# zpaq/zpaq

Hardware: AMD Instinct MI355X
Metric: compress MB/s + bit-identical ratio, -m5 over 1024x1 MiB blocks (higher is better)
Workload: dtype int32

## Files before the change

### profiles/unit_isa.py

```python
#!/usr/bin/env python3
import collections, os, re, subprocess, sys, tempfile
ROOT = os.path.dirname(os.path.dirname(os.path.abspath(__file__)))
sys.path.insert(0, ROOT)


def classify(op):
    if op.startswith("s_waitcnt"): return "s_waitcnt"
    if op.startswith("s_nop"): return "s_nop"
    if op.startswith(("s_cbranch", "s_branch", "s_setpc", "s_swappc", "s_call")): return "branch"
    if op.startswith(("global_", "buffer_", "flat_", "scratch_")): return "vmem"
    if op.startswith("ds_"): return "lds"
    if op.startswith("s_load") or op.startswith("s_buffer"): return "smem"
    if op.startswith("s_"): return "salu"
    if op.startswith("v_"): return "valu"
    return "other"


def main():
    import zpaq_amd as z
    from zpaq_amd import corpus, prebuild
    method = sys.argv[1] if len(sys.argv) > 1 else "3"
    kind = sys.argv[2] if len(sys.argv) > 2 else "lcg"
    bs = int(sys.argv[3]) if len(sys.argv) > 3 else 1 << 18
    mode = int(sys.argv[4]) if len(sys.argv) > 4 else 0
# ... 4 lines not shown
    src, key = prebuild.pipe_source_and_key(header, mode)
    inc = os.path.join(ROOT, "zpaq_amd", "csrc", "device")
    with tempfile.TemporaryDirectory() as td:
        hip = os.path.join(td, "k.hip")
        open(hip, "w").write(src)
        subprocess.run([prebuild.HIPCC, "--offload-arch=gfx950", "-O3", "-std=c++17", "-Wno-unused-label", "-mllvm",
                        "-simplifycfg-sink-common=false", "-I", inc, "--genco", hip, "-o", os.path.join(td, "k.hsaco"),
                        "-save-temps"], cwd=td, check=True, stdout=subprocess.DEVNULL, stderr=subprocess.DEVNULL)
        asm = open(os.path.join(td, "k-hip-amdgcn-amd-amdhsa-gfx950.s")).read()
    names = {0: "HCOMP", 1: "ROW", 2: "light", 3: "ICM map", 4: "ISSE map", 5: "MIX"}
    lk = re.search(r"LIGHT_KIND\[\d+\] = \{([^}]*)\}", src)
    light_kinds = [int(x) for x in lk.group(1).split(",")] if lk else []
    lname = {2: "CONS", 3: "CM", 4: "MATCH", 5: "AVG", 6: "MIX2", 7: "SSE", 8: "CODER", 9: "CM bits", 10: "MIX2 bits", 11: "SSE bits"}
    print(f"chain of method {method} ({kind}, {bs} B blocks), n = {header[6]} components, shape {mode}; key {key}")
    print(f"{'unit':28s} {'loop':>6s} {'per bit':>8s}   valu  salu  vmem   lds  wait  branch  nop   (instructions of the per-byte loop nest, static, all paths)")
    for m in re.finditer(r"^(_ZN3zpq17pipe_persist_unitIN7zpq_gen6ChainPELi(\d+)ELi(\d+)EEEvRKNS_8PipeArgsEjii):[^\n]*\n(.*?)^\.Lfunc_end", asm, re.S | re.M):
        kindn, role, body = int(m.group(2)), int(m.group(3)), m.group(4)
        lines = body.split("\n")
        heads = [(i, int(re.search(r"Depth=(\d+)", l).group(1))) for i, l in enumerate(lines) if "Loop Header: Depth=" in l]
        best = None
        for hi, (i, d) in enumerate(heads):
            if d < 2:
                continue
            j = next((i2 for i2, d2 in heads[hi + 1:] if d2 <= d), len(lines))
            ops = [l.split()[0] for l in lines[i:j] if re.match(r"^\s+[a-z_0-9]+(\s|$)", l) and not l.strip().startswith((";", "."))]
            if best is None or len(ops) > len(best[0]):
                best = (ops, d)
        if best is None:
            continue
        ops = best[0]
        c = collections.Counter(classify(o) for o in ops)
        tag = names.get(kindn, "?")
        if kindn == 2 and role < len(light_kinds):
            tag = lname.get(light_kinds[role], "light")
        print(f"{tag + ' (role %d)' % role:28s} {len(ops):6d} {len(ops) / 8:8.1f}   {c['valu']:4d}  {c['salu']:4d}  {c['vmem']:4d}  {c['lds']:4d}  {c['s_waitcnt']:4d}  {c['branch']:6d}  {c['s_nop']:3d}")


if __name__ == "__main__":
    main()
```

### zpaq_amd/csrc/device/pipe_kernel.h

```cpp
#pragma once
#ifndef ZPQ_LANE_VM
#define ZPQ_LANE_VM 1
#endif
#include "spec_kernel.h"

namespace zpq {

typedef __attribute__((address_space(1))) short g_i16;
typedef __attribute__((address_space(1))) unsigned short g_u16;

#ifdef ZPQ_TRACE
struct PipeTraceScope {
  unsigned long long* rec;
  __device__ __forceinline__ PipeTraceScope(const PipeArgs& a, int kernel) : rec(nullptr) {
    if (a.trace && threadIdx.x == 0) {
      rec = a.trace + 4ull * ((unsigned long long)a.trace_base + blockIdx.x);
      unsigned hw, xcc;
      asm volatile("s_getreg_b32 %0, hwreg(HW_REG_HW_ID)" : "=s"(hw));
      asm volatile("s_getreg_b32 %0, hwreg(HW_REG_XCC_ID)" : "=s"(xcc));
      rec[0] = ((unsigned long long)(unsigned)kernel << 56) | ((unsigned long long)((unsigned)a.step & 0xFFFFFFu) << 32) |
               (unsigned long long)(blockIdx.x + a.wg0);
      rec[1] = ((unsigned long long)xcc << 32) | hw;
      rec[2] = __builtin_amdgcn_s_memrealtime();
    }
// ... 125 lines not shown
  __device__ __forceinline__ g_u128& p(int i, unsigned k) const {
    return *(g_u128*)(gb + (unsigned)Chain::PIPE_OFF_P + ((((slot * N + i) * C + k) * G + gl) << 4));
  }
  __device__ __forceinline__ g_u32& state(int w) const {
    return *(g_u32*)(gb + (unsigned)Chain::PIPE_OFF_STATE + (((unsigned)w * G + gl) << 2));
  }
  __device__ __forceinline__ unsigned off_ctx(int ci, unsigned k) const { return (unsigned)Chain::PIPE_OFF_CTX + ((((slot * Chain::PIPE_NCTX + ci) * C + k) * G + gl) << 2); }
  __device__ __forceinline__ unsigned off_bh(int ri, unsigned k) const { return (unsigned)Chain::PIPE_OFF_BH + ((((slot * Chain::PIPE_NROW + ri) * C + k) * G + gl) << 3); }
  __device__ __forceinline__ unsigned off_p(int i, unsigned k) const { return (unsigned)Chain::PIPE_OFF_P + ((((slot * N + i) * C + k) * G + gl) << 4); }
  __device__ __forceinline__ void put_ctx(int ci, unsigned k, unsigned v) const {
    if constexpr (WT) pipe_wt_store4(gb, off_ctx(ci, k), v); else ctx(ci, k) = v;
  }
  __device__ __forceinline__ void put_bh(int ri, unsigned k, const uint2& v) const {
    if constexpr (WT) pipe_wt_store8(gb, off_bh(ri, k), v); else bh(ri, k) = v;
  }
  __device__ __forceinline__ void put_bh_half(int ri, unsigned k, unsigned half, unsigned v) const {
    if constexpr (WT) pipe_wt_store4(gb, off_bh(ri, k) + 4u * half, v); else *(g_u32*)(gb + off_bh(ri, k) + 4u * half) = v;
  }
  __device__ __forceinline__ void put_p(int i, unsigned k, const uint4& v) const {
    if constexpr (WT) pipe_wt_store16(gb, off_p(i, k), v); else p(i, k) = v;
  }
  __device__ __forceinline__ void put_p64(int i, unsigned k, unsigned half, const uint2& v) const {
    if constexpr (WT) pipe_wt_store8(gb, off_p(i, k) + 8u * half, v); else *(g_u64v*)((g_u8*)&p(i, k) + 8u * half) = v;
  }
  __device__ __forceinline__ void put_p16(int i, unsigned k, unsigned B, int v) const {
    if constexpr (WT) pipe_wt_store2(gb, off_p(i, k) + 2u * B, (unsigned)v & 0xFFFFu); else *(g_i16*)((g_u8*)&p(i, k) + 2u * B) = (short)v;
  }
  __device__ __forceinline__ void put_state(int w, unsigned v) const {
    if constexpr (WT) pipe_wt_store4(gb, (unsigned)Chain::PIPE_OFF_STATE + (((unsigned)w * G + gl) << 2), v); else state(w) = v;
  }
  __device__ __forceinline__ g_u32& A32(unsigned off) const { return *(g_u32*)(arena + off); }
  __device__ __forceinline__ g_u8& A8(unsigned off) const { return *(g_u8*)(arena + off); }
  __device__ __forceinline__ g_u128& A128(unsigned off) const { return *(g_u128*)(arena + off); }
  __device__ __forceinline__ unsigned byte_at(unsigned k) const { return in[k0 + k]; }
  __device__ __forceinline__ unsigned next(unsigned k) const { return min(k + 1u, nb - 1u); }
};

__device__ __forceinline__ int pipe_p_get(const uint4& v, int B) {
  const unsigned w = B < 2 ? v.x : (B < 4 ? v.y : (B < 6 ? v.z : v.w));
  return (int)(short)(unsigned short)(w >> (16 * (B & 1)));
}
struct PipeP8 {
  unsigned w[4] = {0, 0, 0, 0};
  __device__ __forceinline__ void set(int B, int v) { w[B >> 1] |= ((unsigned)v & 0xFFFFu) << (16 * (B & 1)); }
  __device__ __forceinline__ uint4 get() const { return make_uint4(w[0], w[1], w[2], w[3]); }
};
// ... 1798 lines not shown
  __shared__ PipeSquash squash;
  const int lane = threadIdx.x & 63;
  const unsigned ngroups = (a.nblocks + Chain::PIPE_G - 1u) / Chain::PIPE_G;
  const unsigned wg = blockIdx.x + a.wg0;
  squash.load(a.tb, lane);
  __syncthreads();
  static_for<0, Chain::NMIXR>([&](auto rc) __attribute__((always_inline)) {
    constexpr int r = decltype(rc)::value;
    constexpr int I = Chain::MIX_COMP[r], QL = Chain::MIX_QL[r], first = Chain::MIX_FIRST[r];
    constexpr int PPW = 64 / QL, BPW = PPW / 8;
    static_assert(QL <= 8 && BPW >= 1 && (int)Chain::PIPE_G % BPW == 0, "MIX bit lanes: a block's 8 positions share a wavefront");
    constexpr int WPG = (int)Chain::PIPE_G / BPW;
    if (wg < (unsigned)first * ngroups || wg >= (unsigned)(first + WPG) * ngroups) return;
    const unsigned wi = wg - (unsigned)first * ngroups;
    const unsigned g = wi / (unsigned)WPG, sub = wi % (unsigned)WPG;
    const unsigned pair = (unsigned)lane / QL, q = (unsigned)lane % QL, B = pair & 7u;
    PipeLane<Chain> L;
    L.open(a, pipe_opaque(g * Chain::PIPE_G + sub * BPW + (pair >> 3)), Chain::P_LEVEL[I]);
    if (L.chunk < 0 || !pipe_any(L.nb > 0)) return;
    pipe_mix_bits_unit<Chain, r>(L, q, B, squash);
  });
}

template <class Chain, int r, int NH, class SQ>
__device__ __forceinline__ void pipe_mix_unit(PipeLane<Chain>& L, unsigned q, unsigned half, const SQ& squash) {
  constexpr int I = Chain::MIX_COMP[r], QL = Chain::MIX_QL[r];
  constexpr CompK c = Chain::comp[I];
  constexpr int m = (int)c.a3, J = (int)c.a2, ci = Chain::P_CTX[I];
  constexpr int NQ = (m + 3) / 4, TAIL = m % 4, NB = 8 / NH;
  static_assert(NQ <= QL, "MIX lane group");
  constexpr bool batch = c.a5 == 255u && c.mask0 >= 255u;
  static_assert(NH == 1 || (NH == 2 && batch), "a byte is split over lane groups only when its 8 rows are distinct");
  if (!L.nb) return;
  constexpr bool FULL = c.stride >= 4u * (unsigned)QL;
  const bool act = FULL || q < (unsigned)NQ;
  const bool tail = !FULL && TAIL != 0 && q == (unsigned)(NQ - 1);
  const unsigned qoff = 16u * (act ? q : 0u);
  bool have[4];
  int tin[4];
#pragma unroll
  for (int x = 0; x < 4; ++x) {
    const int t = (int)q * 4 + x;
    have[x] = t < m;
    tin[x] = J + (have[x] ? t : 0);
  }
  auto c8_of = [&](unsigned bytev, int b) __attribute__((always_inline)) -> unsigned {
    if constexpr (NH == 1) return pipe_c8(bytev, b);
    else return ((half ? 16u : 1u) << b) | ((half ? bytev : bytev >> 4) >> (4 - b));
  };
  auto y_of = [&](unsigned bytev, int b) __attribute__((always_inline)) -> int {
    if constexpr (NH == 1) return pipe_y(bytev, b);
    else return (int)(((half ? bytev : bytev >> 4) >> (3 - b)) & 1u);
  };
  auto row_of = [&](unsigned hh, unsigned bytev, int b) __attribute__((always_inline)) -> unsigned {
    return (unsigned)c.t0 + 4u * __umul24((hh + (c8_of(bytev, b) & c.a5)) & c.mask0, (unsigned)c.stride) + qoff;
  };
  unsigned h = L.ctx(ci, 0), byte = L.byte_at(0);
  const unsigned k1 = L.next(0);
  unsigned h1 = L.ctx(ci, k1), byte1 = L.byte_at(k1);
  auto inputs = [&](int x, unsigned kk) __attribute__((always_inline)) -> uint4 {
    const uint4 v = L.p(tin[x], kk);
    const unsigned mk = have[x] ? 0xFFFFFFFFu : 0u;
    if constexpr (NH == 1) return make_uint4(v.x & mk, v.y & mk, v.z & mk, v.w & mk);
    else return make_uint4((half ? v.z : v.x) & mk, (half ? v.w : v.y) & mk, 0u, 0u);
  };
  uint4 pv[4], pv1[4];
#pragma unroll
  for (int x = 0; x < 4; ++x) { pv[x] = inputs(x, 0); pv1[x] = inputs(x, k1); }
  uint4 w[NB];
  unsigned rowc[NB];
#pragma unroll
  for (int B = 0; B < NB; ++B) rowc[B] = row_of(h, byte, B);
  if constexpr (batch) {
#pragma unroll
    for (int B = 0; B < NB; ++B) w[B] = *(g_u128a4*)(L.arena + rowc[B]);
  }
  for (unsigned k = 0; k < L.nb; ++k) {
    const unsigned k2 = min(k + 2u, L.nb - 1u);
    const unsigned h2 = L.ctx(ci, k2), byte2 = L.byte_at(k2);
    uint4 pv2[4];
#pragma unroll
    for (int x = 0; x < 4; ++x) pv2[x] = inputs(x, k2);
    unsigned rown[NB];
#pragma unroll
    for (int B = 0; B < NB; ++B) rown[B] = row_of(h1, byte1, B);
    const bool same = h1 == h;
    const bool late = !same && (((h1 - h) & c.mask0) < 256u || ((h - h1) & c.mask0) < 256u);
    uint4 wn[NB], nw[NB];
    if constexpr (batch) {
      if (!late) {
#pragma unroll
        for (int B = 0; B < NB; ++B) wn[B] = *(g_u128a4*)(L.arena + rown[B]);
      }
    }
    PipeP8 out;
#pragma unroll
    for (int B = 0; B < NB; ++B) {
      const unsigned row = rowc[B];
      if constexpr (!batch) w[B] = *(g_u128a4*)(L.arena + row);
      const int w0 = (int)w[B].x, w1 = (int)w[B].y, w2 = (int)w[B].z, w3 = (int)w[B].w;
      const int p0 = pipe_p_get(pv[0], B), p1 = pipe_p_get(pv[1], B), p2 = pipe_p_get(pv[2], B), p3 = pipe_p_get(pv[3], B);
      const int dot = __mul24(w0 >> 8, p0) + __mul24(w1 >> 8, p1) + __mul24(w2 >> 8, p2) + __mul24(w3 >> 8, p3);
      const int pr = sp_clamp2k(pipe_group_sum<QL>(dot) >> 8);
      out.set(B, pr);
      const int err = __mul24(y_of(byte, B) * 32767 - squash(pr), (int)c.a4) >> 4;
      nw[B].x = (unsigned)sp_clamp512k(w0 + ((__mul24(err, p0) + (1 << 12)) >> 13));
      nw[B].y = (unsigned)sp_clamp512k(w1 + ((__mul24(err, p1) + (1 << 12)) >> 13));
      nw[B].z = (unsigned)sp_clamp512k(w2 + ((__mul24(err, p2) + (1 << 12)) >> 13));
      nw[B].w = (unsigned)sp_clamp512k(w3 + ((__mul24(err, p3) + (1 << 12)) >> 13));
      if constexpr (FULL) *(g_u128a4*)(L.arena + row) = nw[B];
      else if (act && !tail) *(g_u128a4*)(L.arena + row) = nw[B];
      if constexpr (TAIL != 0 && !FULL) {
        if (tail) {
          L.A32(row) = nw[B].x;
          if constexpr (TAIL >= 2) L.A32(row + 4u) = nw[B].y;
          if constexpr (TAIL >= 3) L.A32(row + 8u) = nw[B].z;
        }
      }
    }
    if (q == 0) {
      if constexpr (NH == 1) L.put_p(I, k, out.get());
      else L.put_p64(I, k, half, make_uint2(out.w[0], out.w[1]));
    }
    if constexpr (batch) {
      if constexpr (NH == 2) {
        if (pipe_any(late)) pipe_stores_done();
      }
      if (late) {
#pragma unroll
        for (int B = 0; B < NB; ++B) wn[B] = *(g_u128a4*)(L.arena + rown[B]);
      }
#pragma unroll
      for (int B = 0; B < NB; ++B) {
        const bool fw = same && rown[B] == rowc[B];
        w[B].x = fw ? nw[B].x : wn[B].x; w[B].y = fw ? nw[B].y : wn[B].y;
        w[B].z = fw ? nw[B].z : wn[B].z; w[B].w = fw ? nw[B].w : wn[B].w;
      }
    }
    h = h1; byte = byte1; h1 = h2; byte1 = byte2;
#pragma unroll
    for (int B = 0; B < NB; ++B) rowc[B] = rown[B];
#pragma unroll
    for (int x = 0; x < 4; ++x) { pv[x] = pv1[x]; pv1[x] = pv2[x]; }
  }
}

struct PipeW3 { unsigned x, y, z; };
typedef __attribute__((address_space(1))) PipeW3 g_w3;

__device__ __forceinline__ int pipe_sext24(unsigned v) { return (int)(v << 8) >> 8; }
__device__ __forceinline__ void pipe_unpack4(const PipeW3& d, int& w0, int& w1, int& w2, int& w3) {
  w0 = pipe_sext24(d.x);
  w1 = pipe_sext24((d.x >> 24) | (d.y << 8));
  w2 = pipe_sext24((d.y >> 16) | (d.z << 16));
  w3 = (int)d.z >> 8;
}
__device__ __forceinline__ PipeW3 pipe_pack4(int w0, int w1, int w2, int w3) {
  PipeW3 d;
  d.x = ((unsigned)w0 & 0xFFFFFFu) | ((unsigned)w1 << 24);
  d.y = (((unsigned)w1 >> 8) & 0xFFFFu) | ((unsigned)w2 << 16);
  d.z = (((unsigned)w2 >> 16) & 0xFFu) | ((unsigned)w3 << 8);
  return d;
}

__device__ __forceinline__ constexpr unsigned pipe_mix_pstride(unsigned m) {
  const unsigned need = 12u * ((m + 3u) / 4u);
// ... 200 lines not shown
```

### zpaq_amd/csrc/device/pipe_persist.h

```cpp
#pragma once
#include "pipe_kernel.h"

#if !defined(ZPQ_EMU)
#ifndef ZPQ_PERSIST_LDS_BYTES
#error "the generated source defines ZPQ_PERSIST_LDS_BYTES before it includes pipe_persist.h"
#endif
namespace zpq { __shared__ __attribute__((aligned(16))) unsigned char persist_lds[ZPQ_PERSIST_LDS_BYTES]; }
#endif

namespace zpq {

struct PipeRO {
  int dt[1024];
  unsigned short dt2k[256];
  PipeSquash squash;
  PipeStretch stretch;
  unsigned char ns[1024];
};

#ifdef ZPQ_EMU
#define ZPQ_PERSIST_LDS(bytes) ((unsigned char*)emu::wg_lds(bytes))
__device__ __forceinline__ unsigned pipe_prog_load(const unsigned* p) { return *(volatile const unsigned*)p; }
__device__ __forceinline__ void pipe_prog_add(unsigned* p) { *(volatile unsigned*)p = *(volatile unsigned*)p + 1u; }
__device__ __forceinline__ void pipe_flag_set(unsigned* p, unsigned v) { *(volatile unsigned*)p = v; }
// ... 104 lines not shown

template <class Chain>
__device__ __forceinline__ void pipe_publish(unsigned* prog, int unit, int lane) {
  pipe_drain_stores();
  if (lane == 0) pipe_prog_add(prog + unit);
}

template <class Chain, int kind, int role>
__device__ __attribute__((noinline)) void pipe_persist_unit(const PipeArgs& a, unsigned g, int lane, int SLOT) {
  unsigned char* const lds = ZPQ_PERSIST_LDS(Chain::PS_LDS_BYTES);
  const PipeRO& ro = *(const PipeRO*)lds;
  const int sub = Chain::PS_SUB[SLOT], unit = Chain::PS_UNIT[SLOT];
  constexpr unsigned G = Chain::PIPE_G;
  unsigned* const prog = pipe_uniform(a.prog + (unsigned long long)g * (unsigned)Chain::PS_NUNIT);
  const unsigned nchunks = a.group_chunks[g];
  unsigned char* const priv = lds + Chain::PS_LDS[SLOT];
  PipeLane<Chain> L;
  unsigned q = 0, B = 0, mix_bl = 0;
  if constexpr (kind == 0) {
    constexpr int HL = Chain::HCOMP_LANES < (int)G ? Chain::HCOMP_LANES : (int)G;
    const bool mine = lane < HL;
    L.bind(a, g, (unsigned)sub * HL + (mine ? (unsigned)lane : 0u), mine);
  } else if constexpr (kind == 5) {
    constexpr int QL = Chain::MIX_QL[role];
    if constexpr (Chain::MIX_BITS != 0) {
      constexpr int BPW = 64 / QL / 8;
      const unsigned pair = (unsigned)lane / QL;
      q = (unsigned)lane % QL; B = pair & 7u;
      L.bind(a, g, pipe_opaque((unsigned)sub * BPW + (pair >> 3)), true);
    } else {
      constexpr int NH = Chain::PS_MIX_NH;
      constexpr int BPW = 64 / (QL * NH) < (int)G ? 64 / (QL * NH) : (int)G;
      const unsigned bl = (unsigned)lane / (QL * NH);
      q = (unsigned)lane % QL; B = ((unsigned)lane / QL) % NH;
      mix_bl = bl;
      const bool okl = bl < (unsigned)BPW;
      L.bind(a, g, (unsigned)sub * BPW + (okl ? bl : 0u), okl);
    }
  } else if constexpr (kind == 2 && Chain::LIGHT_KIND[role < 0 ? 0 : role] >= PK_CM_BITS) {
    B = (unsigned)lane & 7u;
    const unsigned gl = (unsigned)sub * 8u + ((unsigned)lane >> 3);
    L.bind(a, g, gl < G ? gl : 0u, gl < G);
  } else if constexpr (kind == 1 && pipe_row_in_halves<Chain>(role < 0 ? 0 : role)) {
    L.bind(a, g, (unsigned)lane & 31u, true);
  } else {
    const bool okl = (unsigned)lane < G;
    L.bind(a, g, okl ? (unsigned)lane : 0u, okl);
  }
  if (!L.live) L.idle();
  L.gb = pipe_uniform(L.gb);
  unsigned long long t_wait = 0, t_work = 0, t_mark = a.trace ? pipe_clock() : 0ull;
  for (unsigned c = 0; c < nchunks; ++c) {
    if (!pipe_wait<Chain>(a, prog, c, lane, SLOT)) return;
// ... 17 lines not shown
        }
        if (pipe_any(L.nb > 0)) pipe_icm_unit<Chain, Chain::ICM_COMP[role], PipeStretchFull, PipeAhead<Chain>::value>(L, (unsigned*)priv, PipeStretchFull{st}, lane, c == 0, false);
      } else {
        if (pipe_any(L.nb > 0)) pipe_icm_unit<Chain, Chain::ICM_COMP[role], PipeStretch, PipeAhead<Chain>::value>(L, (unsigned*)priv, ro.stretch, lane, c == 0, false);
      }
    } else if constexpr (kind == 4) {
      if constexpr (PipeSmallChain<Chain>::value) {
        unsigned short* const sq = (unsigned short*)(priv + 512u * G * 4u);
        if (c == 0) {
          for (int i = lane; i < 4096; i += 64) sq[i] = a.tb->squash[i];
          (void)pipe_any(true);
        }
        if (pipe_any(L.nb > 0)) pipe_isse_unit<Chain, Chain::ISSE_COMP[role], PipeSquashFull, PipeAhead<Chain>::value>(L, (unsigned*)priv, PipeSquashFull{sq}, lane, c == 0, false);
      } else {
        if (pipe_any(L.nb > 0)) pipe_isse_packed_unit<Chain, Chain::ISSE_COMP[role], PipeSquash, PipeAhead<Chain>::value>(L, (unsigned*)priv, ro.squash, lane, c == 0);
      }
    } else if constexpr (kind == 5) {
      if (pipe_any(L.nb > 0)) {
        if constexpr (Chain::MIX_BITS != 0) pipe_mix_bits_unit<Chain, role>(L, q, B, ro.squash);
        else if constexpr (PipeMixPacked<Chain>::of(role)) {
          constexpr int QL = Chain::MIX_QL[role], NH = Chain::PS_MIX_NH, BPW = 64 / (QL * NH) < (int)G ? 64 / (QL * NH) : (int)G;
          pipe_mix_packed_unit<Chain, role, PipeMixLdsRows<Chain>::of(role), BPW, NH>(L, q, B, mix_bl < (unsigned)BPW ? mix_bl : 0u, (unsigned*)priv, c == 0, ro.squash);
        }
        else pipe_mix_unit<Chain, role, Chain::PS_MIX_NH>(L, q, B, ro.squash);
      }
    } else {
      constexpr int lk = Chain::LIGHT_KIND[role], I = Chain::LIGHT_COMP[role];
      if constexpr (lk == PK_CODER) {
        if constexpr (PipeCoderFast<Chain>::value) pipe_coder_fast<Chain, (PipeAhead<Chain>::value > 0 ? PipeAhead<Chain>::value : 1)>(L, a, (unsigned*)priv, lane, c == 0);
        else pipe_coder<Chain>(L, a, ro.squash);
      } else if (pipe_any(L.nb > 0)) {
        if constexpr (lk == PK_CONS) pipe_cons<Chain, I>(L);
        else if constexpr (lk == PK_CM) {
          if constexpr (pipe_light_lds_words<Chain>(lk, I) != 0u) pipe_cm_lds<Chain, I>(L, (unsigned*)priv, ro.stretch, ro.dt, lane, c == 0);
          else pipe_cm<Chain, I>(L, ro.stretch, ro.dt);
        }
        else if constexpr (lk == PK_MATCH) pipe_match_any<Chain, I>(L, ro.stretch, ro.dt2k);
        else if constexpr (lk == PK_AVG) pipe_avg<Chain, I>(L);
        else if constexpr (lk == PK_MIX2) {
          if constexpr (pipe_light_lds_words<Chain>(lk, I) != 0u) pipe_mix2_lds<Chain, I>(L, (unsigned*)priv, ro.squash, lane, c == 0);
          else pipe_mix2<Chain, I>(L, ro.squash);
        }
        else if constexpr (lk == PK_SSE) pipe_sse<Chain, I>(L, ro.stretch, ro.dt);
        else if constexpr (lk == PK_CM_BITS) pipe_cm_bits<Chain, I>(L, B, ro.stretch, ro.dt);
        else if constexpr (lk == PK_MIX2_BITS) pipe_mix2_bits<Chain, I>(L, B, ro.squash);
        else if constexpr (lk == PK_SSE_BITS) pipe_sse_bits<Chain, I>(L, B, ro.stretch, ro.dt);
      }
// ... 42 lines not shown
```

### zpaq_amd/csrc/host/codegen.cpp

```cpp
#include "codegen.hpp"

#include <cstdio>
#include <cstdlib>
#include <cstring>
#include <map>
#include <mutex>
#include <set>
#include <sstream>
#include <algorithm>

namespace zpq {

namespace {

struct Insn { int pc, len, op; };

std::string src_expr(int k, int imm) {
  switch (k) {
    case 0: return "a";
    case 1: return "b";
    case 2: return "c";
    case 3: return "d";
    case 4: return "(unsigned)M[b & MMASK]";
    case 5: return "(unsigned)M[c & MMASK]";
// ... 264 lines not shown
       "extern \"C\" __global__ __launch_bounds__(64 * zpq_gen::Chain::WAVES) void zpq_spec_decode(const zpq::BlockJob* jobs, "
       "zpq::BlockResult* res, unsigned nblocks, const zpq::DeviceTables* tb) {\n"
       "  " << body << "<zpq_gen::Chain, true>(jobs, res, nblocks, tb);\n}\n";
  source = o.str();
  return true;
}

PipeOptions pipe_options(int variant) {
  PipeOptions o;
  o.mode = variant ? 1 : 0;
  o.chunk = variant == 2 ? 2048 : 0;
  o.wide = variant == 3;
  return o;
}

static const int kPersistRoBytes = 4096 + 512 + 2688 + (2016 * 4 + 512) + 1024;
static const int kPersistLdsCap = 163840 - 512;
static uint32_t mix_pstride(uint32_t m) {
  const uint32_t need = 12u * ((m + 3u) / 4u);
  uint32_t p = 16u;
  while (p < need) p *= 2u;
  return p;
}
static void plan_persistent(const zpq_plan& plan, PipeLayout& L, int lds_rows_wish, bool halves) {
  const CompDesc* comp = plan.comps();
  const PlanHeader& ph = plan.hdr();
  const int n = L.n, G = L.G;
  enum { K_CONS = 2, K_CM, K_MATCH, K_AVG, K_MIX2, K_SSE, K_CODER, K_CM_BITS, K_MIX2_BITS, K_SSE_BITS };
  L.persist_ok = false;
  L.ps_slots.clear(); L.ps_deps.clear();
  int nunit = 1;
  std::vector<int> row_unit(n, -1), p_unit(n, -1);
  for (int i = 0; i < n; ++i) {
    if (L.row[i] >= 0) row_unit[i] = nunit++;
    p_unit[i] = nunit++;
  }
  const int coder_unit = nunit++;
  L.ps_nunit = nunit;
  std::vector<int> unit_waves(nunit, 0);
  std::vector<PipeLayout::Slot> slots;
  static const float ondie_w = [] { const char* v = getenv("ZPAQ_AMD_PACK_ONDIE_WEIGHT"); return v ? (float)atof(v) : 1.0f; }();
  static const float stream_w = [] { const char* v = getenv("ZPAQ_AMD_PACK_STREAM_WEIGHT"); return v ? (float)atof(v) : 1.0f; }();
  static const float match_lines = [] { const char* v = getenv("ZPAQ_AMD_PACK_MATCH_LINES"); return v ? (float)atof(v) : 3.0f; }();
  const float ctx_l = G * 4 / 128.f, bh_l = G * 8 / 128.f, p_l = G * 16 / 128.f;
  auto add = [&](int kind, int role, int sub, int unit, int lds, float cost, float lines = 0.f, float stream_lines = 0.f) {
    PipeLayout::Slot s; s.kind = kind; s.role = role; s.sub = sub; s.unit = unit; s.lds = (lds + 255) & ~255; s.cost = cost;
    s.lines = lines + stream_w * stream_lines;
// ... 37 lines not shown
    int code_role = (int)r;
    for (size_t r2 = 0; r2 < r; ++r2) if (L.light[r2] == L.light[r]) { code_role = (int)r2; break; }
    int lds = 0;
    if ((k == K_CM || (k == K_MIX2 && comp[i].mask0 != 0u)) && comp[i].mask0 + 1u <= 512u && comp[i].mask0 >= 3u) lds = (int)(comp[i].mask0 + 1u) * G * 4;
    float lines = 0.f;
    if (!lds) {
      const float wcm = line_weight(4ull * (comp[i].mask0 + 1ull));
      if (k == K_CM) lines = 2.f * G * wcm;
      else if (k == K_CM_BITS) lines = 2.f * 8 * wcm;
      else if (k == K_MATCH) lines = match_lines * G;
      else if (k == K_MIX2 && comp[i].mask0 != 0u) lines = 8.f * G * wcm;
      else if (k == K_MIX2_BITS) lines = 8.f * 8 * wcm;
      else if (k == K_SSE) lines = 8.f * G * wcm;
      else if (k == K_SSE_BITS) lines = 8.f * 8 * wcm;
    }
    const bool bits = k >= K_CM_BITS;
    float sl = (k == K_CODER ? p_l : p_l + ctx_l) + (k == K_MIX2 || k == K_MIX2_BITS || k == K_AVG ? 2.f * p_l : (k == K_SSE || k == K_SSE_BITS ? p_l : 0.f));
    if (bits) sl *= 8.f * 8.f / (float)(G * 8);
    if (k == K_CODER && L.ps_coder_fast) lds = 4096 * 4;
    add(2, code_role, L.light_sub[r], k == K_CODER ? coder_unit : p_unit[i], lds, lds && k != K_CODER ? 0.9f : lc[k < 12 ? k : 0], lines, sl);
  }
  for (size_t r = 0; r < L.icm.size(); ++r) add(3, (int)r, 0, p_unit[L.icm[r]], 256 * G * 4 + (small && L.ps_icm_full ? 65536 : 0), 1.1f, 0.f, bh_l + p_l);
  for (size_t r = 0; r < L.isse.size(); ++r) add(4, (int)r, 0, p_unit[L.isse[r]], small ? 512 * G * 4 + 8192 : 256 * G * 4 + 64 * G * 4, 1.5f, 0.f, bh_l + 2.f * p_l);
  L.ps_mix_nh = 1;
  if (halves && !L.mix_bits && !L.mix.empty()) {
    bool ok = true;
    for (size_t r = 0; r < L.mix.size(); ++r) {
      const CompDesc& c = comp[L.mix[r]];
      ok = ok && c.a5 == 255u && c.mask0 >= 255u && L.mix_ql[r] * 2 <= 64;
    }
    if (ok) L.ps_mix_nh = 2;
  }
  L.mix_lds_rows.assign(L.mix.size(), 0);
  for (size_t r = 0; r < L.mix.size(); ++r) {
    const int nw = L.mix_bits ? L.mix_waves_of(L.mix_ql[r]) : std::max(1, G * L.mix_ql[r] * L.ps_mix_nh / 64);
    int lds = 0;
    const CompDesc& c = comp[L.mix[r]];
    if (!L.mix_bits && L.mix_packed[r] && c.mask0 + 1u <= 256u && lds_rows_wish > 0) {
      const int rows = std::min<int>(lds_rows_wish, (int)(c.mask0 + 1u));
      const int nq = ((int)c.a3 + 3) / 4, bpw = std::max(1, std::min(G, 64 / (L.mix_ql[r] * L.ps_mix_nh)));
      L.mix_lds_rows[r] = rows;
      lds = 3 * rows * nq * bpw * 4;
    }
    const float groups_per_wave = 64.f / (float)L.mix_ql[r];
    float lines = groups_per_wave * (L.mix_bits ? 1.f : 8.f / (float)L.ps_mix_nh) * line_weight(4ull * c.stride * (c.mask0 + 1ull));
    if (L.mix_lds_rows[r]) lines *= 1.f / 8.f;
    for (int sub = 0; sub < nw; ++sub)
      add(5, (int)r, sub, p_unit[L.mix[r]], lds, L.mix_bits ? 0.55f : (L.ps_mix_nh == 2 ? 1.7f : (lds ? 1.6f : 2.6f)), lines, (float)c.a3 + ctx_l);
  }
  std::vector<std::vector<int>> producers(nunit);
  auto reads = [&](int u, int v) { if (u != v && std::find(producers[u].begin(), producers[u].end(), v) == producers[u].end()) producers[u].push_back(v); };
  for (int i = 0; i < n; ++i) {
    const CompDesc& c = comp[i];
    const int u = p_unit[i];
    if (L.row[i] >= 0) { reads(row_unit[i], 0); reads(u, row_unit[i]); }
    else if (L.ctx[i] >= 0) reads(u, 0);
    switch (c.type) {
      case C_ISSE: reads(u, p_unit[c.a2]); break;
      case C_AVG: reads(u, p_unit[c.a1]); reads(u, p_unit[c.a2]); break;
      case C_MIX2: reads(u, p_unit[c.a2]); reads(u, p_unit[c.a3]); break;
      case C_SSE: reads(u, p_unit[c.a2]); break;
      case C_MIX: for (unsigned t = 0; t < c.a3; ++t) reads(u, p_unit[c.a2 + t]); break;
      default: break;
    }
  }
  reads(coder_unit, p_unit[n - 1]);
  reads(coder_unit, 0);
  std::vector<std::vector<PipeLayout::Dep>> unit_deps(nunit);
  for (int u = 0; u < nunit; ++u)
    for (int v : producers[u]) {
      unit_deps[u].push_back({v, 0, unit_waves[v]});
// ... 235 lines not shown
  L.coder_state = L.nstate; L.nstate += 4;
  const uint64_t hbytes = 4ull * (ph.hmask + 1);
  L.hcomp_h_lds = hbytes <= 8192;
  L.hcomp_lanes = 64;
  if (L.hcomp_h_lds) while (L.hcomp_lanes > 8 && hbytes * L.hcomp_lanes > 65536) L.hcomp_lanes /= 2;
  const uint64_t C = (uint64_t)L.C, S = (uint64_t)L.S, G = (uint64_t)L.G;
  uint64_t off = 0;
  L.off_ctx = off;   off += S * (uint64_t)std::max(L.nctx, 1) * C * G * 4;
  L.off_bh = off;    off += S * (uint64_t)std::max(L.nrow, 1) * C * G * 8;
  L.off_p = off;     off += S * (uint64_t)n * C * G * 16;
  L.off_state = off; off += (uint64_t)L.nstate * G * 4;
  L.group_bytes = (off + 4095) & ~4095ull;
  if (L.group_bytes >= (1ull << 32)) { why_not = "stream buffer of a block group exceeds 4 GiB"; return false; }
  L.mix_packed.assign(L.mix.size(), 0);
  static const bool packed_off = [] { const char* v = getenv("ZPAQ_AMD_MIX_PACKED"); return !(v && v[0] == '1'); }();
  for (size_t r = 0; r < L.mix.size(); ++r) {
    const CompDesc& c = comp[L.mix[r]];
    const uint32_t ps = mix_pstride(c.a3);
    if (!packed_off && !L.mix_bits && c.a5 == 255u && c.mask0 >= 255u && c.a3 >= 3u && ps <= 4u * c.stride && (ps < 4u * c.stride || c.mask0 + 1u <= 256u))
      L.mix_packed[r] = 1;
  }
  static const int rows_forced = [] { const char* v = getenv("ZPAQ_AMD_MIX_LDS_ROWS"); return v ? atoi(v) : -1; }();
  static const bool halves_wanted = [] { const char* v = getenv("ZPAQ_AMD_MIX_HALVES"); return !(v && v[0] == '0'); }();
  plan_persistent(plan, L, 0, false);
  bool halves = false;
  if (L.persist_ok && halves_wanted) {
    PipeLayout T = L;
    plan_persistent(plan, T, 0, true);
    if (T.persist_ok && T.ps_mix_nh == 2 && T.ps_wpg <= L.ps_wpg) { L = T; halves = true; }
  }
  if (L.persist_ok) {
    const int wpg0 = L.ps_wpg;
    for (int wish : {128, 64, 32}) {
      if (rows_forced >= 0 && wish != rows_forced) continue;
      PipeLayout T = L;
      plan_persistent(plan, T, wish, halves);
      bool any = false;
      for (int v : T.mix_lds_rows) any = any || v != 0;
      if (!any) break;
      if (T.persist_ok && T.ps_wpg <= wpg0) { L = T; break; }
    }
  }
  return true;
}

bool generate_pipe_source(const zpq_plan& plan, const PipeOptions& opt, std::string& source, std::string& why_not) {
  PipeLayout L;
  if (!pipe_layout(plan, opt, L, why_not)) return false;
  const PlanHeader& ph = plan.hdr();
  const int n = L.n;
  const CompDesc* comp = plan.comps();
  std::ostringstream o;
  o << "// generated by zpaq_amd codegen v" << kCodegenVersion << " (pipelined encoder) -- do not edit\n"
       "#define ZPQ_PERSIST_LDS_BYTES " << (L.persist_ok && opt.persist && opt.chunk != 2048 ? L.ps_lds_bytes : 16) << "\n"
       "#include \"pipe_persist.h\"\n"
       "namespace zpq_gen {\n"
       "struct Chain {\n";
  int nmix = 0, nsse = 0;
  std::ostringstream comps;
// ... 63 lines not shown
         "  static constexpr bool PIPE_PERSIST = true;\n"
         "  static constexpr int PS_MIX_NH = " << L.ps_mix_nh << ";\n"
         "  static constexpr bool HCOMP_M_LDS = " << (L.hcomp_m_lds ? "true" : "false") << ";\n"
         "  static constexpr int PS_AHEAD = " << L.ps_ahead << ";\n"
         "  static constexpr bool PS_ROW_RING = " << (L.ps_row_ring ? "true" : "false") << ";\n"
         "  static constexpr bool PS_CODER_FAST = " << (L.ps_coder_fast ? "true" : "false") << ", PS_SMALL = " << (L.ps_small ? "true" : "false") << ";\n"
      << (L.ps_small && !L.ps_row_halves ? "  static constexpr bool PS_ROW_HALVES = false;\n" : "")
      << (L.ps_small && !L.ps_icm_full ? "  static constexpr bool PS_ICM_FULL = false;\n" : "")
      << "";
    o <<
         "  static constexpr int PS_WAVES = " << L.ps_waves << ", PS_WPG = " << L.ps_wpg << ", PS_NSLOT = " << L.ps_slots.size()
      << ", PS_NUNIT = " << L.ps_nunit << ", PS_LDS_BYTES = " << L.ps_lds_bytes << ";\n";
    arr("PS_KIND", kind.data(), (int)kind.size());
    arr("PS_ROLE", role.data(), (int)role.size());
    arr("PS_SUB", sub.data(), (int)sub.size());
    arr("PS_UNIT", unit.data(), (int)unit.size());
    arr("PS_LDS", ldso.data(), (int)ldso.size());
    arr("PS_DEP0", dep0.data(), (int)dep0.size());
    arr("PS_NDEP", ndep.data(), (int)ndep.size());
    arr("PS_DEP_UNIT", du.data(), (int)du.size());
    arr("PS_DEP_LAG", dl.data(), (int)dl.size());
    arr("PS_DEP_MULT", dm.data(), (int)dm.size());
    arr("MIX_LDS_ROWS", L.mix_lds_rows.data(), (int)L.mix_lds_rows.size());
    o << "};\n";
  }
  o << "}  // namespace zpq_gen\n";
  if (L.persist_ok && opt.persist && opt.chunk != 2048)
    o << "extern \"C\" __global__ __launch_bounds__(" << 64 * L.ps_waves << ") void zpq_pipe_persist(zpq::PipeArgs a) {\n"
         "  zpq::pipe_persist_body<zpq_gen::ChainP>(a);\n}\n";
  else
    o << "#ifdef ZPQ_EMU\nextern \"C\" void zpq_pipe_persist(zpq::PipeArgs) {}\n#endif\n";
  o << "extern \"C\" __global__ __launch_bounds__(256) void zpq_pipe_repack(zpq::PipeArgs a) {\n"
       "  zpq::pipe_repack_body<zpq_gen::Chain>(a);\n}\n";
  const char* names[6] = {"hcomp", "rows", "light", "icm", "isse", "mix"};
  for (int k = 0; k < 6; ++k)
    o << "extern \"C\" __global__ __launch_bounds__(64) void zpq_pipe_" << names[k] << "(zpq::PipeArgs a) {\n"
         "  ZPQ_PIPE_TRACE(a, " << k << ");\n"
         "  zpq::pipe_" << names[k] << "_body<zpq_gen::Chain>(a);\n}\n";
  source = o.str();
  return true;
}

bool generate_pcomp_source(const U8* code, size_t len, int ph, int pm, std::string& source, std::string& why_not) {
  if (len < 1 || len > 65535) { why_not = "empty or oversized PCOMP"; return false; }
  if (ph > 28 || pm > 30) { why_not = "PCOMP arrays too large"; return false; }
  std::ostringstream o;
// ... 25 lines not shown
```

### zpaq_amd/csrc/host/codegen.hpp

```cpp
#pragma once
#include <string>
#include <utility>
#include <vector>

#include "../device/plan.hpp"
#include "common.hpp"

namespace zpq {

static const int kCodegenVersion = 6;

bool generate_spec_source(const zpq_plan& plan, int waves, std::string& source, std::string& why_not, int shape = 0);
int team_threads(const zpq_plan& plan);

struct PipeOptions {
  int mode = 0;
  int chunk = 0;
  int group = 0;
  bool persist = true;
  bool wide = false;
};
static const int kPipeVariants = 4;
PipeOptions pipe_options(int variant);

// ... 25 lines not shown
    int role = 0;
    int sub = 0;
    int unit = 0;
    int lds = 0;
    int lds_off = 0;
    float cost = 0;
    float lines = 0;
  };
  struct Dep { int unit, lag, mult; };
  bool persist_ok = false;
  std::string persist_why;
  int ps_waves = 0;
  int ps_wpg = 0;
  int ps_nunit = 0;
  int ps_lds_bytes = 0;
  bool ps_coder_fast = false;
  bool ps_row_ring = false;
  int ps_ahead = 0;
  bool ps_wide = false;
  bool ps_icm_full = false;
  bool ps_row_halves = false;
  bool ps_small = false;
  int ps_mix_nh = 1;
  std::vector<Slot> ps_slots;
  std::vector<std::vector<Dep>> ps_deps;
  int light_threads() const { return 64; }
  int mix_waves_of(int ql) const { return mix_bits ? G * ql / 8 : ql; }
  int mix_waves_per_group() const { int s = 0; for (int q : mix_ql) s += mix_waves_of(q); return s; }
  int mix_threads() const { return mix_bits ? 64 : G; }
};
bool pipe_layout(const zpq_plan& plan, const PipeOptions& opt, PipeLayout& out, std::string& why_not);
bool generate_pipe_source(const zpq_plan& plan, const PipeOptions& opt, std::string& source, std::string& why_not);

bool generate_pcomp_source(const U8* code, size_t len, int ph, int pm, std::string& source, std::string& why_not);

std::string spec_cache_key(const std::string& source);

}
```

Before: 386.9.

## Split MIX bytes over four lane groups and allow five weights per lane

The persistent pipeline's MIX unit can now split each byte's 8 bit-rows across four lane groups instead of two. It can also give each lane five weights instead of four when that halves the lane group and the padded row stride allows it. The planner tries NH=4 first, then NH=2, and emits per-role lane-group sizes and words-per-lane tables. This aims to shorten each lane's serial bit chain and cut the lanes spent per mixer. The cost is extra 32-bit partial stores of predictions and more units to schedule. The unit_isa profiling script is also changed to find loop extents more precisely and skip spin-wait loops.

```diff
diff --git a/profiles/unit_isa.py b/profiles/unit_isa.py
--- a/profiles/unit_isa.py
+++ b/profiles/unit_isa.py
@@ -50,8 +50,14 @@
         for hi, (i, d) in enumerate(heads):
             if d < 2:
                 continue
-            j = next((i2 for i2, d2 in heads[hi + 1:] if d2 <= d), len(lines))
+            name = next((re.match(r"^\.L(BB\d+_\d+):", lines[k]).group(1) for k in range(i, max(i - 4, -1), -1) if re.match(r"^\.LBB\d+_\d+:", lines[k])), None)
+            if name is None:
+                continue
+            last = max((k for k, l in enumerate(lines) if re.search(r"(Header=|Parent Loop )%s\b" % name, l)), default=i)
+            j = next((k for k in range(last + 1, len(lines)) if re.match(r"^(\.LBB\d+_\d+:|; %bb\.\d+:)", lines[k])), len(lines))
             ops = [l.split()[0] for l in lines[i:j] if re.match(r"^\s+[a-z_0-9]+(\s|$)", l) and not l.strip().startswith((";", "."))]
+            if "s_sleep" in ops:
+                continue
             if best is None or len(ops) > len(best[0]):
                 best = (ops, d)
         if best is None:
diff --git a/zpaq_amd/csrc/device/pipe_kernel.h b/zpaq_amd/csrc/device/pipe_kernel.h
--- a/zpaq_amd/csrc/device/pipe_kernel.h
+++ b/zpaq_amd/csrc/device/pipe_kernel.h
@@ -171,6 +171,9 @@
   }
   __device__ __forceinline__ void put_p64(int i, unsigned k, unsigned half, const uint2& v) const {
     if constexpr (WT) pipe_wt_store8(gb, off_p(i, k) + 8u * half, v); else *(g_u64v*)((g_u8*)&p(i, k) + 8u * half) = v;
+  }
+  __device__ __forceinline__ void put_p32(int i, unsigned k, unsigned part, unsigned v) const {
+    if constexpr (WT) pipe_wt_store4(gb, off_p(i, k) + 4u * part, v); else *(g_u32*)((g_u8*)&p(i, k) + 4u * part) = v;
   }
   __device__ __forceinline__ void put_p16(int i, unsigned k, unsigned B, int v) const {
     if constexpr (WT) pipe_wt_store2(gb, off_p(i, k) + 2u * B, (unsigned)v & 0xFFFFu); else *(g_i16*)((g_u8*)&p(i, k) + 2u * B) = (short)v;
@@ -2015,35 +2018,48 @@
   });
 }
 
-template <class Chain, int r, int NH, class SQ>
-__device__ __forceinline__ void pipe_mix_unit(PipeLane<Chain>& L, unsigned q, unsigned half, const SQ& squash) {
-  constexpr int I = Chain::MIX_COMP[r], QL = Chain::MIX_QL[r];
+template <class Chain, int r, int NH, int QL = Chain::MIX_QL[r], int WPL = 4, class SQ>
+__device__ __forceinline__ void pipe_mix_unit(PipeLane<Chain>& L, unsigned q, unsigned part, const SQ& squash) {
+  constexpr int I = Chain::MIX_COMP[r];
   constexpr CompK c = Chain::comp[I];
   constexpr int m = (int)c.a3, J = (int)c.a2, ci = Chain::P_CTX[I];
-  constexpr int NQ = (m + 3) / 4, TAIL = m % 4, NB = 8 / NH;
+  constexpr int NQ = (m + WPL - 1) / WPL, TAIL = m % WPL, NB = 8 / NH;
   static_assert(NQ <= QL, "MIX lane group");
+  static_assert(WPL == 4 || (WPL == 5 && c.stride >= 5u * (unsigned)QL), "five words a lane: the group's words lie in the padded row");
   constexpr bool batch = c.a5 == 255u && c.mask0 >= 255u;
-  static_assert(NH == 1 || (NH == 2 && batch), "a byte is split over lane groups only when its 8 rows are distinct");
+  static_assert(NH == 1 || ((NH == 2 || NH == 4) && batch), "a byte is split over lane groups only when its 8 rows are distinct");
   if (!L.nb) return;
-  constexpr bool FULL = c.stride >= 4u * (unsigned)QL;
+  constexpr bool FULL = c.stride >= (unsigned)(WPL * QL);
   const bool act = FULL || q < (unsigned)NQ;
   const bool tail = !FULL && TAIL != 0 && q == (unsigned)(NQ - 1);
-  const unsigned qoff = 16u * (act ? q : 0u);
-  bool have[4];
-  int tin[4];
-#pragma unroll
-  for (int x = 0; x < 4; ++x) {
-    const int t = (int)q * 4 + x;
+  const unsigned qoff = 4u * WPL * (act ? q : 0u);
+  bool have[WPL];
+  int tin[WPL];
+#pragma unroll
+  for (int x = 0; x < WPL; ++x) {
+    const int t = (int)q * WPL + x;
     have[x] = t < m;
     tin[x] = J + (have[x] ? t : 0);
   }
+  auto load_row = [&](unsigned row, unsigned (&d)[WPL]) __attribute__((always_inline)) {
+    const uint4 v = *(g_u128a4*)(L.arena + row);
+    d[0] = v.x; d[1] = v.y; d[2] = v.z; d[3] = v.w;
+    if constexpr (WPL == 5) d[4] = L.A32(row + 16u);
+  };
+  auto store_row = [&](unsigned row, const unsigned (&d)[WPL]) __attribute__((always_inline)) {
+    *(g_u128a4*)(L.arena + row) = make_uint4(d[0], d[1], d[2], d[3]);
+    if constexpr (WPL == 5) L.A32(row + 16u) = d[4];
+  };
+  const unsigned lead = 1u << (NB * part), sh = 8u - NB * (part + 1u);
   auto c8_of = [&](unsigned bytev, int b) __attribute__((always_inline)) -> unsigned {
     if constexpr (NH == 1) return pipe_c8(bytev, b);
-    else return ((half ? 16u : 1u) << b) | ((half ? bytev : bytev >> 4) >> (4 - b));
+    else if constexpr (NH == 2) return ((part ? 16u : 1u) << b) | ((part ? bytev : bytev >> 4) >> (4 - b));
+    else return (lead << b) | ((bytev >> sh) >> (NB - b));
   };
   auto y_of = [&](unsigned bytev, int b) __attribute__((always_inline)) -> int {
     if constexpr (NH == 1) return pipe_y(bytev, b);
-    else return (int)(((half ? bytev : bytev >> 4) >> (3 - b)) & 1u);
+    else if constexpr (NH == 2) return (int)(((part ? bytev : bytev >> 4) >> (3 - b)) & 1u);
+    else return (int)(((bytev >> sh) >> (NB - 1 - b)) & 1u);
   };
   auto row_of = [&](unsigned hh, unsigned bytev, int b) __attribute__((always_inline)) -> unsigned {
     return (unsigned)c.t0 + 4u * __umul24((hh + (c8_of(bytev, b) & c.a5)) & c.mask0, (unsigned)c.stride) + qoff;
@@ -2052,89 +2068,89 @@
   const unsigned k1 = L.next(0);
   unsigned h1 = L.ctx(ci, k1), byte1 = L.byte_at(k1);
   auto inputs = [&](int x, unsigned kk) __attribute__((always_inline)) -> uint4 {
+    const unsigned mk = have[x] ? 0xFFFFFFFFu : 0u;
+    if constexpr (NH == 4) return make_uint4(*(const g_u32*)((const g_u8*)&L.p(tin[x], kk) + 4u * part) & mk, 0u, 0u, 0u);
     const uint4 v = L.p(tin[x], kk);
-    const unsigned mk = have[x] ? 0xFFFFFFFFu : 0u;
     if constexpr (NH == 1) return make_uint4(v.x & mk, v.y & mk, v.z & mk, v.w & mk);
-    else return make_uint4((half ? v.z : v.x) & mk, (half ? v.w : v.y) & mk, 0u, 0u);
-  };
-  uint4 pv[4], pv1[4];
-#pragma unroll
-  for (int x = 0; x < 4; ++x) { pv[x] = inputs(x, 0); pv1[x] = inputs(x, k1); }
-  uint4 w[NB];
+    else return make_uint4((part ? v.z : v.x) & mk, (part ? v.w : v.y) & mk, 0u, 0u);
+  };
+  uint4 pv[WPL], pv1[WPL];
+#pragma unroll
+  for (int x = 0; x < WPL; ++x) { pv[x] = inputs(x, 0); pv1[x] = inputs(x, k1); }
+  unsigned w[NB][WPL];
   unsigned rowc[NB];
 #pragma unroll
   for (int B = 0; B < NB; ++B) rowc[B] = row_of(h, byte, B);
   if constexpr (batch) {
 #pragma unroll
-    for (int B = 0; B < NB; ++B) w[B] = *(g_u128a4*)(L.arena + rowc[B]);
+    for (int B = 0; B < NB; ++B) load_row(rowc[B], w[B]);
   }
   for (unsigned k = 0; k < L.nb; ++k) {
     const unsigned k2 = min(k + 2u, L.nb - 1u);
     const unsigned h2 = L.ctx(ci, k2), byte2 = L.byte_at(k2);
-    uint4 pv2[4];
-#pragma unroll
-    for (int x = 0; x < 4; ++x) pv2[x] = inputs(x, k2);
+    uint4 pv2[WPL];
+#pragma unroll
+    for (int x = 0; x < WPL; ++x) pv2[x] = inputs(x, k2);
     unsigned rown[NB];
 #pragma unroll
     for (int B = 0; B < NB; ++B) rown[B] = row_of(h1, byte1, B);
     const bool same = h1 == h;
     const bool late = !same && (((h1 - h) & c.mask0) < 256u || ((h - h1) & c.mask0) < 256u);
-    uint4 wn[NB], nw[NB];
+    unsigned wn[NB][WPL], nw[NB][WPL];
     if constexpr (batch) {
       if (!late) {
 #pragma unroll
-        for (int B = 0; B < NB; ++B) wn[B] = *(g_u128a4*)(L.arena + rown[B]);
+        for (int B = 0; B < NB; ++B) load_row(rown[B], wn[B]);
       }
     }
     PipeP8 out;
 #pragma unroll
     for (int B = 0; B < NB; ++B) {
       const unsigned row = rowc[B];
-      if constexpr (!batch) w[B] = *(g_u128a4*)(L.arena + row);
-      const int w0 = (int)w[B].x, w1 = (int)w[B].y, w2 = (int)w[B].z, w3 = (int)w[B].w;
-      const int p0 = pipe_p_get(pv[0], B), p1 = pipe_p_get(pv[1], B), p2 = pipe_p_get(pv[2], B), p3 = pipe_p_get(pv[3], B);
-      const int dot = __mul24(w0 >> 8, p0) + __mul24(w1 >> 8, p1) + __mul24(w2 >> 8, p2) + __mul24(w3 >> 8, p3);
+      if constexpr (!batch) load_row(row, w[B]);
+      int p[WPL];
+      int dot = 0;
+#pragma unroll
+      for (int x = 0; x < WPL; ++x) { p[x] = pipe_p_get(pv[x], B); dot += __mul24((int)w[B][x] >> 8, p[x]); }
       const int pr = sp_clamp2k(pipe_group_sum<QL>(dot) >> 8);
       out.set(B, pr);
       const int err = __mul24(y_of(byte, B) * 32767 - squash(pr), (int)c.a4) >> 4;
-      nw[B].x = (unsigned)sp_clamp512k(w0 + ((__mul24(err, p0) + (1 << 12)) >> 13));
-      nw[B].y = (unsigned)sp_clamp512k(w1 + ((__mul24(err, p1) + (1 << 12)) >> 13));
-      nw[B].z = (unsigned)sp_clamp512k(w2 + ((__mul24(err, p2) + (1 << 12)) >> 13));
-      nw[B].w = (unsigned)sp_clamp512k(w3 + ((__mul24(err, p3) + (1 << 12)) >> 13));
-      if constexpr (FULL) *(g_u128a4*)(L.arena + row) = nw[B];
-      else if (act && !tail) *(g_u128a4*)(L.arena + row) = nw[B];
+#pragma unroll
+      for (int x = 0; x < WPL; ++x) nw[B][x] = (unsigned)sp_clamp512k((int)w[B][x] + ((__mul24(err, p[x]) + (1 << 12)) >> 13));
+      if constexpr (FULL) store_row(row, nw[B]);
+      else if (act && !tail) store_row(row, nw[B]);
       if constexpr (TAIL != 0 && !FULL) {
         if (tail) {
-          L.A32(row) = nw[B].x;
-          if constexpr (TAIL >= 2) L.A32(row + 4u) = nw[B].y;
-          if constexpr (TAIL >= 3) L.A32(row + 8u) = nw[B].z;
+#pragma unroll
+          for (int x = 0; x < TAIL; ++x) L.A32(row + 4u * x) = nw[B][x];
         }
       }
     }
     if (q == 0) {
       if constexpr (NH == 1) L.put_p(I, k, out.get());
-      else L.put_p64(I, k, half, make_uint2(out.w[0], out.w[1]));
+      else if constexpr (NH == 2) L.put_p64(I, k, part, make_uint2(out.w[0], out.w[1]));
+      else L.put_p32(I, k, part, out.w[0]);
     }
     if constexpr (batch) {
-      if constexpr (NH == 2) {
+      if constexpr (NH >= 2) {
         if (pipe_any(late)) pipe_stores_done();
       }
       if (late) {
 #pragma unroll
-        for (int B = 0; B < NB; ++B) wn[B] = *(g_u128a4*)(L.arena + rown[B]);
+        for (int B = 0; B < NB; ++B) load_row(rown[B], wn[B]);
       }
 #pragma unroll
       for (int B = 0; B < NB; ++B) {
         const bool fw = same && rown[B] == rowc[B];
-        w[B].x = fw ? nw[B].x : wn[B].x; w[B].y = fw ? nw[B].y : wn[B].y;
-        w[B].z = fw ? nw[B].z : wn[B].z; w[B].w = fw ? nw[B].w : wn[B].w;
+#pragma unroll
+        for (int x = 0; x < WPL; ++x) w[B][x] = fw ? nw[B][x] : wn[B][x];
       }
     }
     h = h1; byte = byte1; h1 = h2; byte1 = byte2;
 #pragma unroll
     for (int B = 0; B < NB; ++B) rowc[B] = rown[B];
 #pragma unroll
-    for (int x = 0; x < 4; ++x) { pv[x] = pv1[x]; pv1[x] = pv2[x]; }
+    for (int x = 0; x < WPL; ++x) { pv[x] = pv1[x]; pv1[x] = pv2[x]; }
   }
 }
 
diff --git a/zpaq_amd/csrc/device/pipe_persist.h b/zpaq_amd/csrc/device/pipe_persist.h
--- a/zpaq_amd/csrc/device/pipe_persist.h
+++ b/zpaq_amd/csrc/device/pipe_persist.h
@@ -150,13 +150,14 @@
     const bool mine = lane < HL;
     L.bind(a, g, (unsigned)sub * HL + (mine ? (unsigned)lane : 0u), mine);
   } else if constexpr (kind == 5) {
-    constexpr int QL = Chain::MIX_QL[role];
     if constexpr (Chain::MIX_BITS != 0) {
+      constexpr int QL = Chain::MIX_QL[role];
       constexpr int BPW = 64 / QL / 8;
       const unsigned pair = (unsigned)lane / QL;
       q = (unsigned)lane % QL; B = pair & 7u;
       L.bind(a, g, pipe_opaque((unsigned)sub * BPW + (pair >> 3)), true);
     } else {
+      constexpr int QL = Chain::PS_MIX_QL[role];
       constexpr int NH = Chain::PS_MIX_NH;
       constexpr int BPW = 64 / (QL * NH) < (int)G ? 64 / (QL * NH) : (int)G;
       const unsigned bl = (unsigned)lane / (QL * NH);
@@ -220,7 +221,7 @@
           constexpr int QL = Chain::MIX_QL[role], NH = Chain::PS_MIX_NH, BPW = 64 / (QL * NH) < (int)G ? 64 / (QL * NH) : (int)G;
           pipe_mix_packed_unit<Chain, role, PipeMixLdsRows<Chain>::of(role), BPW, NH>(L, q, B, mix_bl < (unsigned)BPW ? mix_bl : 0u, (unsigned*)priv, c == 0, ro.squash);
         }
-        else pipe_mix_unit<Chain, role, Chain::PS_MIX_NH>(L, q, B, ro.squash);
+        else pipe_mix_unit<Chain, role, Chain::PS_MIX_NH, Chain::PS_MIX_QL[role], Chain::PS_MIX_WPL[role]>(L, q, B, ro.squash);
       }
     } else {
       constexpr int lk = Chain::LIGHT_KIND[role], I = Chain::LIGHT_COMP[role];
diff --git a/zpaq_amd/csrc/host/codegen.cpp b/zpaq_amd/csrc/host/codegen.cpp
--- a/zpaq_amd/csrc/host/codegen.cpp
+++ b/zpaq_amd/csrc/host/codegen.cpp
@@ -310,7 +310,14 @@
   while (p < need) p *= 2u;
   return p;
 }
-static void plan_persistent(const zpq_plan& plan, PipeLayout& L, int lds_rows_wish, bool halves) {
+static void mix_lane_group(uint32_t m, uint32_t stride, int& ql, int& wpl) {
+  auto lanes = [m](uint32_t words) { const uint32_t need = (m + words - 1u) / words; int q = 1; while ((uint32_t)q < need) q *= 2; return q; };
+  ql = lanes(4u); wpl = 4;
+  const int q5 = lanes(5u);
+  if (q5 < ql && 5u * (uint32_t)q5 <= stride) { ql = q5; wpl = 5; }
+}
+
+static void plan_persistent(const zpq_plan& plan, PipeLayout& L, int lds_rows_wish, int nh) {
   const CompDesc* comp = plan.comps();
   const PlanHeader& ph = plan.hdr();
   const int n = L.n, G = L.G;
@@ -394,18 +401,24 @@
   }
   for (size_t r = 0; r < L.icm.size(); ++r) add(3, (int)r, 0, p_unit[L.icm[r]], 256 * G * 4 + (small && L.ps_icm_full ? 65536 : 0), 1.1f, 0.f, bh_l + p_l);
   for (size_t r = 0; r < L.isse.size(); ++r) add(4, (int)r, 0, p_unit[L.isse[r]], small ? 512 * G * 4 + 8192 : 256 * G * 4 + 64 * G * 4, 1.5f, 0.f, bh_l + 2.f * p_l);
+  L.ps_mix_ql = L.mix_ql;
+  L.ps_mix_wpl.assign(L.mix.size(), 4);
+  if (L.mode == 0 && !L.mix_bits)
+    for (size_t r = 0; r < L.mix.size(); ++r)
+      if (!L.mix_packed[r]) mix_lane_group(comp[L.mix[r]].a3, comp[L.mix[r]].stride, L.ps_mix_ql[r], L.ps_mix_wpl[r]);
   L.ps_mix_nh = 1;
-  if (halves && !L.mix_bits && !L.mix.empty()) {
+  if (nh > 1 && !L.mix_bits && !L.mix.empty()) {
     bool ok = true;
     for (size_t r = 0; r < L.mix.size(); ++r) {
       const CompDesc& c = comp[L.mix[r]];
-      ok = ok && c.a5 == 255u && c.mask0 >= 255u && L.mix_ql[r] * 2 <= 64;
-    }
-    if (ok) L.ps_mix_nh = 2;
+      ok = ok && c.a5 == 255u && c.mask0 >= 255u && L.ps_mix_ql[r] * nh <= 64 && (nh == 2 || !L.mix_packed[r]);
+    }
+    if (ok) L.ps_mix_nh = nh;
   }
   L.mix_lds_rows.assign(L.mix.size(), 0);
   for (size_t r = 0; r < L.mix.size(); ++r) {
-    const int nw = L.mix_bits ? L.mix_waves_of(L.mix_ql[r]) : std::max(1, G * L.mix_ql[r] * L.ps_mix_nh / 64);
+    const int QL = L.ps_mix_ql[r];
+    const int nw = L.mix_bits ? L.mix_waves_of(L.mix_ql[r]) : std::max(1, G * QL * L.ps_mix_nh / 64);
     int lds = 0;
     const CompDesc& c = comp[L.mix[r]];
     if (!L.mix_bits && L.mix_packed[r] && c.mask0 + 1u <= 256u && lds_rows_wish > 0) {
@@ -414,11 +427,12 @@
       L.mix_lds_rows[r] = rows;
       lds = 3 * rows * nq * bpw * 4;
     }
-    const float groups_per_wave = 64.f / (float)L.mix_ql[r];
+    const float groups_per_wave = 64.f / (float)(L.mix_bits ? L.mix_ql[r] : QL);
     float lines = groups_per_wave * (L.mix_bits ? 1.f : 8.f / (float)L.ps_mix_nh) * line_weight(4ull * c.stride * (c.mask0 + 1ull));
     if (L.mix_lds_rows[r]) lines *= 1.f / 8.f;
+    const float cost = L.mix_bits ? 0.55f : (L.ps_mix_nh == 4 ? 1.0f : (L.ps_mix_nh == 2 ? 1.7f : (lds ? 1.6f : 2.6f)));
     for (int sub = 0; sub < nw; ++sub)
-      add(5, (int)r, sub, p_unit[L.mix[r]], lds, L.mix_bits ? 0.55f : (L.ps_mix_nh == 2 ? 1.7f : (lds ? 1.6f : 2.6f)), lines, (float)c.a3 + ctx_l);
+      add(5, (int)r, sub, p_unit[L.mix[r]], lds, cost, lines, (float)c.a3 + ctx_l);
   }
   std::vector<std::vector<int>> producers(nunit);
   auto reads = [&](int u, int v) { if (u != v && std::find(producers[u].begin(), producers[u].end(), v) == producers[u].end()) producers[u].push_back(v); };
@@ -700,19 +714,23 @@
   }
   static const int rows_forced = [] { const char* v = getenv("ZPAQ_AMD_MIX_LDS_ROWS"); return v ? atoi(v) : -1; }();
   static const bool halves_wanted = [] { const char* v = getenv("ZPAQ_AMD_MIX_HALVES"); return !(v && v[0] == '0'); }();
-  plan_persistent(plan, L, 0, false);
-  bool halves = false;
+  static const int nh_max_ab = [] { const char* v = getenv("ZPAQ_AMD_MIX_NH_MAX"); return v ? atoi(v) : 4; }();
+  plan_persistent(plan, L, 0, 1);
+  int nh = 1;
   if (L.persist_ok && halves_wanted) {
-    PipeLayout T = L;
-    plan_persistent(plan, T, 0, true);
-    if (T.persist_ok && T.ps_mix_nh == 2 && T.ps_wpg <= L.ps_wpg) { L = T; halves = true; }
+    for (int want : {4, 2}) {
+      if (want > nh_max_ab || (want == 4 && L.mode != 0)) continue;
+      PipeLayout T = L;
+      plan_persistent(plan, T, 0, want);
+      if (T.persist_ok && T.ps_mix_nh == want && T.ps_wpg <= L.ps_wpg) { L = T; nh = want; break; }
+    }
   }
   if (L.persist_ok) {
     const int wpg0 = L.ps_wpg;
     for (int wish : {128, 64, 32}) {
       if (rows_forced >= 0 && wish != rows_forced) continue;
       PipeLayout T = L;
-      plan_persistent(plan, T, wish, halves);
+      plan_persistent(plan, T, wish, nh);
       bool any = false;
       for (int v : T.mix_lds_rows) any = any || v != 0;
       if (!any) break;
@@ -822,6 +840,8 @@
     arr("PS_DEP_LAG", dl.data(), (int)dl.size());
     arr("PS_DEP_MULT", dm.data(), (int)dm.size());
     arr("MIX_LDS_ROWS", L.mix_lds_rows.data(), (int)L.mix_lds_rows.size());
+    arr("PS_MIX_QL", L.ps_mix_ql.data(), (int)L.ps_mix_ql.size());
+    arr("PS_MIX_WPL", L.ps_mix_wpl.data(), (int)L.ps_mix_wpl.size());
     o << "};\n";
   }
   o << "}  // namespace zpq_gen\n";
diff --git a/zpaq_amd/csrc/host/codegen.hpp b/zpaq_amd/csrc/host/codegen.hpp
--- a/zpaq_amd/csrc/host/codegen.hpp
+++ b/zpaq_amd/csrc/host/codegen.hpp
@@ -71,6 +71,7 @@
   bool ps_row_halves = false;
   bool ps_small = false;
   int ps_mix_nh = 1;
+  std::vector<int> ps_mix_ql, ps_mix_wpl;
   std::vector<Slot> ps_slots;
   std::vector<std::vector<Dep>> ps_deps;
   int light_threads() const { return 64; }
```

Result: slower. 359.5, median of 2 (-7.1%).
